# zju3dv/NeuralRecon-W

Hardware: AMD Instinct MI355X
Metric: ray-samples/sec (train step) at 1024 rays x 128 samples (higher is better)
Workload: dtype f16; 1 GPU; brandenburg_gate config (BASELINE.json configs[1]): 1024 rays/GPU x (64 coarse + 64 fine) samples, SDF 8x256 + colour 4x256 + bg NeRF 8x256, 4 outside samples, up_sample_steps 2, render+loss+backward+allreduce+clip+Adam; rays_per_gpu=1024, samples_per_ray=128, global_rays=1024, parallelism=dp1, world_size=1, submission=eager, streams=2, skipped_steps=0

## Files before the change

### neuralrecon-w_amd/csrc/ncw_split.hip

```cpp
#include "ncw_mlp.h"

#ifdef NCW_HALF_F16

namespace {

constexpr int SS_WAVES = 8, SS_TILES = 4;
constexpr int SS_ACT = SS_TILES * 16 * 2 * 1024;
constexpr int SS_GAM = SS_TILES * 3 * 2 * 1024;
constexpr int SB_ACT = SS_TILES * 16 * 1024;

typedef __attribute__((address_space(3))) bf16x8 ss_lfrag;

NCW_DEV bf16x8 ss_gload(const void* w, size_t unit, int lane) {
    return ncw_ld_frag<bf16x8>(w, (size_t)unit, lane);
}

template <int NU>
NCW_DEV void ss_load_half(bf16x8 (&h)[NU], bf16x8 (&l)[NU], const void* w, const void* wlo, int rb_stride, int ob, int u0, int lane) {
#pragma unroll
    for (int q = 0; q < NU; ++q) {
        h[q] = ss_gload(w, (size_t)(u0 + q) * rb_stride + ob, lane);
        l[q] = ss_gload(wlo, (size_t)(u0 + q) * rb_stride + ob, lane);
    }
}

NCW_DEV void ss_split8(const f32x16& v, int t, bf16x8& hi, bf16x8& lo) { ncw_split8(v, t, hi, lo); }

constexpr int SS_RD = 2;
template <int NU>
NCW_DEV void ss_mma(f32x16 (&acc)[SS_TILES], const bf16x8 (&wh)[NU], const bf16x8 (&wl)[NU], const ss_lfrag* in, int upt, int u0) {
    constexpr int NS = (SS_TILES / 2) * NU, RD = SS_RD < NS ? SS_RD : NS, R = RD + 1 < NS ? RD + 1 : NS;
    bf16x8 b[R][4];
    auto ring_read = [&](int s) {
        const ss_lfrag* p0 = in + ((2 * (s / NU) * upt + u0 + s % NU) * 2) * 64;
        const ss_lfrag* p1 = in + (((2 * (s / NU) + 1) * upt + u0 + s % NU) * 2) * 64;
        b[s % R][0] = p0[0]; b[s % R][1] = p0[64];
        b[s % R][2] = p1[0]; b[s % R][3] = p1[64];
    };
#pragma unroll
    for (int s = 0; s < RD; ++s) ring_read(s);
#pragma unroll
    for (int s = 0; s < NS; ++s) {
        if (s + RD < NS) ring_read(s + RD);
        const int tp = 2 * (s / NU), q = s % NU;
        const bf16x8 (&f)[4] = b[s % R];
        acc[tp] = NCW_MFMA_H(wh[q], f[0], acc[tp], 0, 0, 0);
        acc[tp + 1] = NCW_MFMA_H(wh[q], f[2], acc[tp + 1], 0, 0, 0);
        acc[tp] = NCW_MFMA_H(wl[q], f[0], acc[tp], 0, 0, 0);
        acc[tp + 1] = NCW_MFMA_H(wl[q], f[2], acc[tp + 1], 0, 0, 0);
        acc[tp] = NCW_MFMA_H(wh[q], f[1], acc[tp], 0, 0, 0);
        acc[tp + 1] = NCW_MFMA_H(wh[q], f[3], acc[tp + 1], 0, 0, 0);
        __builtin_amdgcn_sched_barrier(0);
    }
}

NCW_DEV f32x16 ss_bias(const float* bp, int ob, int lane) {
    CVec<1> b1;
    load_bias(b1, bp + ob * 32, lane);
    return b1.v[0];
}

NCW_DEV void ss_load_sprime(f32x16& sv, const ncw_h16* __restrict__ st_h, size_t tile, int RB, int rb, int lane) {
    stash_load_block(sv, st_h, tile, RB, rb, lane);
#pragma unroll
    for (int r = 0; r < 16; ++r) sv[r] = 1.f - __builtin_amdgcn_exp2f(sv[r] * -144.26950408889634f);
}

template <int STASH>
NCW_DEV void ss_value_chain(const NcwSdfNet& net, const NcwPoints& src, int64_t n, int64_t tile0, ss_lfrag* abuf, ss_lfrag* gbuf,
                            int lane, int wave, float* __restrict__ sdf, const NcwSdfStash& st) {
    typedef ncw_h16 SE;
    constexpr bool TU = STASH == 0;
    const float bscale = TU ? NCW_TU : 1.f;
    const int L = net.n_layers;
    if (wave < SS_TILES) {
        int64_t p = (tile0 + wave) * 32 + (lane & 31), ray;
        if (p >= n) p = n - 1;
        float xs[3];
        load_point(src, p, xs, ray);
        xs[0] *= net.scale; xs[1] *= net.scale; xs[2] *= net.scale;
        CVec<2> gam;
        freq_encode<2, 3, 6, false>(gam, xs, lane);
        if (STASH == 2) stash_store<2>((SE*)st.gamma, (size_t)(tile0 + wave), gam, lane);
        if (TU) cvec_scale<2>(gam, NCW_TU);
#pragma unroll
        for (int q = 0; q < 3; ++q) {
            bf16x8 hi, lo;
            ss_split8(gam.v[q >> 1], q & 1, hi, lo);
            gbuf[((wave * 3 + q) * 2 + 0) * 64 + lane] = hi;
            gbuf[((wave * 3 + q) * 2 + 1) * 64 + lane] = lo;
        }
    }
    bf16x8 Ah[8], Al[8], Bh[8], Bl[8];
    f32x16 acc[SS_TILES];
    const ss_lfrag* const ain = abuf + lane;
    const ss_lfrag* const gin = gbuf + lane;
    auto epilogue = [&](int l_out) {
        ncw_lds_barrier();
#pragma unroll
        for (int t = 0; t < SS_TILES; ++t) {
            f32x16 yv;
#pragma unroll
            for (int r = 0; r < 16; ++r) yv[r] = softplus_sel<TU>(acc[t][r]);
            if (STASH >= 1) stash_store_block_keep((SE*)st.h[l_out], (size_t)(tile0 + t), 8, wave, yv, lane);
#pragma unroll
            for (int tt = 0; tt < 2; ++tt) {
                bf16x8 hi, lo;
                ss_split8(yv, tt, hi, lo);
                abuf[((t * 16 + 2 * wave + tt) * 2 + 0) * 64 + lane] = hi;
                abuf[((t * 16 + 2 * wave + tt) * 2 + 1) * 64 + lane] = lo;
            }
        }
        ncw_lds_barrier();
    };
    f32x16 bnext;
    {
        bf16x8 w0h[3], w0l[3];
        ss_load_half<3>(w0h, w0l, net.w[0], net.w_lo[0], 8, wave, 0, lane);
        if (L - 1 > 1) ss_load_half<8>(Ah, Al, net.w[1], net.w_lo[1], 8, wave, 0, lane);
        const f32x16 bias = ss_bias(net.b[0], wave, lane) * bscale;
#pragma unroll
        for (int t = 0; t < SS_TILES; ++t) acc[t] = bias;
        ncw_lds_barrier();
        ss_mma<3>(acc, w0h, w0l, gin, 3, 0);
        bnext = ss_bias(net.b[L - 1 > 1 ? 1 : 0], wave, lane);
        epilogue(1);
    }
    for (int l = 1; l < L - 1; ++l) {
        const f32x16 bias = bnext * bscale;
#pragma unroll
        for (int t = 0; t < SS_TILES; ++t) acc[t] = bias;
        ss_load_half<8>(Bh, Bl, net.w[l], net.w_lo[l], 8, wave, 8, lane);
        ss_mma<8>(acc, Ah, Al, ain, 16, 0);
        if (l + 1 < L - 1) ss_load_half<8>(Ah, Al, net.w[l + 1], net.w_lo[l + 1], 8, wave, 0, lane);
        ss_mma<8>(acc, Bh, Bl, ain, 16, 8);
        if (l == net.skip_layer) {
            bf16x8 wgh[3], wgl[3];
            ss_load_half<3>(wgh, wgl, net.w[l], net.w_lo[l], 8, wave, 16, lane);
            ss_mma<3>(acc, wgh, wgl, gin, 3, 0);
        }
        bnext = ss_bias(net.b[l + 1 < L - 1 ? l + 1 : l], wave, lane);
        epilogue(l + 1);
    }
    if (wave < SS_TILES) {
        CVec<1> o;
        load_bias(o, net.b[L - 1], lane);
        if (TU) cvec_scale<1>(o, NCW_TU);
#pragma unroll
        for (int half = 0; half < 2; ++half) {
            bf16x8 wh[8], wl[8];
            ss_load_half<8>(wh, wl, net.w[L - 1], net.w_lo[L - 1], 1, 0, 8 * half, lane);
#pragma unroll
            for (int q = 0; q < 8; ++q) {
                const ss_lfrag* p = ain + ((wave * 16 + 8 * half + q) * 2) * 64;
                const bf16x8 bh = p[0], bl = p[64];
                o.v[0] = NCW_MFMA_H(wh[q], bh, o.v[0], 0, 0, 0);
                o.v[0] = NCW_MFMA_H(wl[q], bh, o.v[0], 0, 0, 0);
                o.v[0] = NCW_MFMA_H(wh[q], bl, o.v[0], 0, 0, 0);
            }
        }
        const int64_t p = (tile0 + wave) * 32 + (lane & 31);
        if (p < n && lane < 32) sdf[p] = o.v[0][0] / (net.scale * bscale);
    }
}

constexpr int S2_TILE = 16 * 2 * 1024;

constexpr int S2_BIAS = 8 * 1024;
typedef __attribute__((address_space(3))) f32x4 ss_lf4;

NCW_DEV void s2_barrier() {
    asm volatile("s_waitcnt lgkmcnt(0)" ::: "memory");
    __builtin_amdgcn_s_barrier();
    asm volatile("" ::: "memory");
}

NCW_DEV f32x16 s2_bias(const ss_lf4* bb, int lane) {
    const ss_lf4* p = bb + (lane >> 5) * 4;
    f32x16 v;
#pragma unroll
    for (int g = 0; g < 4; ++g) {
        const f32x4 t = p[g];
#pragma unroll
        for (int c = 0; c < 4; ++c) v[4 * g + c] = t[c];
    }
    return v;
}

template <int NU>
NCW_DEV void s2_mma_x(f32x16& a, const bf16x8* wh, const bf16x8* wl, const ss_lfrag* xin) {
#pragma unroll
    for (int u = 0; u < NU; ++u) {
        const bf16x8 bh = xin[(u * 2) * 64], bl = xin[(u * 2 + 1) * 64];
        a = NCW_MFMA_H(wh[u], bh, a, 0, 0, 0);
        a = NCW_MFMA_H(wl[u], bh, a, 0, 0, 0);
        a = NCW_MFMA_H(wh[u], bl, a, 0, 0, 0);
    }
}

constexpr int S2_RING = 3;
template <bool PREFETCH, class EPI>
NCW_DEV void s2_segment(f32x16& m, bf16x8 (&wh)[16], bf16x8 (&wl)[16], const ss_lfrag* in, const void* wn, const void* wn_lo, int ob,
                        int lane, EPI&& epi) {
    f32x16 c;
#pragma unroll
    for (int r = 0; r < 16; ++r) c[r] = 0.f;
    constexpr int RD = S2_RING - 1;
    bf16x8 b[S2_RING][2];
#pragma unroll
    for (int q = 0; q < RD; ++q) { b[q][0] = in[(q * 2) * 64]; b[q][1] = in[(q * 2 + 1) * 64]; }
#pragma unroll
    for (int u = 0; u < 16; ++u) {
        if (u + RD < 16) {
            b[(u + RD) % S2_RING][0] = in[((u + RD) * 2) * 64];
            b[(u + RD) % S2_RING][1] = in[((u + RD) * 2 + 1) * 64];
        }
        m = NCW_MFMA_H(wh[u], b[u % S2_RING][0], m, 0, 0, 0);
        c = NCW_MFMA_H(wl[u], b[u % S2_RING][0], c, 0, 0, 0);
        c = NCW_MFMA_H(wh[u], b[u % S2_RING][1], c, 0, 0, 0);
        if (PREFETCH) {
            wh[u] = ss_gload(wn, (size_t)u * 8 + ob, lane);
            wl[u] = ss_gload(wn_lo, (size_t)u * 8 + ob, lane);
        }
        epi(u);
        __builtin_amdgcn_sched_barrier(0);
    }
#pragma unroll
    for (int r = 0; r < 16; ++r) m[r] += c[r];
}

template <bool STASH>
NCW_DEV void s2_epi_step(int u, const f32x16& e, bf16x8& fh, bf16x8& fl, float& ycarry, ss_lfrag* out, int ob, int lane,
                         ncw_h16* __restrict__ st_h, size_t tile) {
    const float y = softplus_sel<!STASH>(e[u]);
    if ((u & 1) == 0) {
        ycarry = y;
    } else {
        ncw_h16 h0, h1, l0, l1;
        ncw_split2(ycarry, y, h0, h1, l0, l1);
        fh[(u & 7) - 1] = h0; fh[u & 7] = h1;
        fl[(u & 7) - 1] = l0; fl[u & 7] = l1;
    }
    if (STASH && (u & 3) == 3) {
        bf16x4 t;
#pragma unroll
        for (int c = 0; c < 4; ++c) t[c] = fh[(u & 7) - 3 + c];
        reinterpret_cast<bf16x4*>(st_h)[((tile * 8 + ob) * 4 + (u >> 2)) * 64 + lane] = t;
    }
    if ((u & 7) == 7) {
        const int unit = 2 * ob + (u >> 3);
        out[(unit * 2 + 0) * 64 + lane] = fh;
        out[(unit * 2 + 1) * 64 + lane] = fl;
    }
}

template <bool STASH>
NCW_DEV void s2_value_chain(const NcwSdfNet& net, const NcwPoints& src, int64_t n, int64_t tile0, ss_lfrag* abuf, ss_lfrag* gbuf,
                            ss_lf4* bbuf, int lane, int wave, float* __restrict__ sdf, const NcwSdfStash& st) {
    typedef ncw_h16 SE;
    const int L = net.n_layers, NL = L - 1;
    const int ob = wave;
    constexpr bool TU = !STASH;
    const float bscale = TU ? NCW_TU : 1.f;
    for (int i = threadIdx.x; i < NL * 64; i += 64 * SS_WAVES) bbuf[i] = reinterpret_cast<const f32x4*>(net.b[i >> 6])[i & 63] * bscale;
    if (wave < SS_TILES) {
        int64_t p = (tile0 + wave) * 32 + (lane & 31), ray;
        if (p >= n) p = n - 1;
        float xs[3];
        load_point(src, p, xs, ray);
        xs[0] *= net.scale; xs[1] *= net.scale; xs[2] *= net.scale;
        CVec<2> gam;
        freq_encode<2, 3, 6, false>(gam, xs, lane);
        if (STASH == 2) stash_store<2>((SE*)st.gamma, (size_t)(tile0 + wave), gam, lane);
        if (TU) cvec_scale<2>(gam, NCW_TU);
#pragma unroll
        for (int q = 0; q < 3; ++q) {
            bf16x8 hi, lo;
            ss_split8(gam.v[q >> 1], q & 1, hi, lo);
            gbuf[((wave * 3 + q) * 2 + 0) * 64 + lane] = hi;
            gbuf[((wave * 3 + q) * 2 + 1) * 64 + lane] = lo;
        }
    }
    bf16x8 wh[16], wl[16];
    f32x16 x, y;
    bf16x8 fh, fl;
    float yc = 0.f;
    auto region = [&](int t) { return abuf + t * (S2_TILE / 16); };
    auto gin = [&](int t) { return gbuf + t * 3 * 2 * 64 + lane; };
    auto bias_of = [&](int l) { return s2_bias(bbuf + (l * 8 + ob) * 8, lane); };
    {
        ss_load_half<3>(reinterpret_cast<bf16x8(&)[3]>(wh[0]), reinterpret_cast<bf16x8(&)[3]>(wl[0]), net.w[0], net.w_lo[0], 8, ob, 0, lane);
        s2_barrier();
        x = bias_of(0);
        y = x;
        s2_mma_x<3>(x, wh, wl, gin(0));
        s2_mma_x<3>(y, wh, wl, gin(1));
#pragma unroll
        for (int u = 0; u < 16; ++u) s2_epi_step<STASH>(u, x, fh, fl, yc, region(0), ob, lane, (SE*)st.h[1], (size_t)tile0);
#pragma unroll
        for (int u = 0; u < 16; ++u) s2_epi_step<STASH>(u, y, fh, fl, yc, region(1), ob, lane, (SE*)st.h[1], (size_t)(tile0 + 1));
        x = bias_of(0);
        y = x;
        s2_mma_x<3>(x, wh, wl, gin(2));
        s2_mma_x<3>(y, wh, wl, gin(3));
        if (NL > 1) ss_load_half<16>(wh, wl, net.w[1], net.w_lo[1], 8, ob, 0, lane);
#pragma unroll
        for (int u = 0; u < 16; ++u) s2_epi_step<STASH>(u, x, fh, fl, yc, region(2), ob, lane, (SE*)st.h[1], (size_t)(tile0 + 2));
        s2_barrier();
    }
    for (int l = 1; l < NL; ++l) {
        const bool more = l + 1 < NL, skip = (l == net.skip_layer);
        bf16x8 gh[3], gl[3];
        if (skip) ss_load_half<3>(gh, gl, net.w[l], net.w_lo[l], 8, ob, 16, lane);
        {
            x = bias_of(l);
            auto epi = [&](int u) { s2_epi_step<STASH>(u, y, fh, fl, yc, region(3), ob, lane, (SE*)st.h[l], (size_t)(tile0 + 3)); };
            s2_segment<false>(x, wh, wl, region(0) + lane, nullptr, nullptr, ob, lane, epi);
            if (skip) s2_mma_x<3>(x, gh, gl, gin(0));
            s2_barrier();
        }
        {
            y = bias_of(l);
            auto epi = [&](int u) { s2_epi_step<STASH>(u, x, fh, fl, yc, region(0), ob, lane, (SE*)st.h[l + 1], (size_t)tile0); };
            s2_segment<false>(y, wh, wl, region(1) + lane, nullptr, nullptr, ob, lane, epi);
            if (skip) s2_mma_x<3>(y, gh, gl, gin(1));
            s2_barrier();
        }
        {
            x = bias_of(l);
            auto epi = [&](int u) { s2_epi_step<STASH>(u, y, fh, fl, yc, region(1), ob, lane, (SE*)st.h[l + 1], (size_t)(tile0 + 1)); };
            s2_segment<false>(x, wh, wl, region(2) + lane, nullptr, nullptr, ob, lane, epi);
            if (skip) s2_mma_x<3>(x, gh, gl, gin(2));
            s2_barrier();
        }
        {
            y = bias_of(l);
            auto epi = [&](int u) { s2_epi_step<STASH>(u, x, fh, fl, yc, region(2), ob, lane, (SE*)st.h[l + 1], (size_t)(tile0 + 2)); };
            s2_segment<true>(y, wh, wl, region(3) + lane, more ? net.w[l + 1] : net.w[l], more ? net.w_lo[l + 1] : net.w_lo[l], ob, lane, epi);
            if (skip) s2_mma_x<3>(y, gh, gl, gin(3));
            s2_barrier();
        }
    }
#pragma unroll
    for (int u = 0; u < 16; ++u) s2_epi_step<STASH>(u, y, fh, fl, yc, region(3), ob, lane, (SE*)st.h[NL], (size_t)(tile0 + 3));
    s2_barrier();
    if (wave < SS_TILES) {
        CVec<1> o;
        load_bias(o, net.b[L - 1], lane);
        if (TU) cvec_scale<1>(o, NCW_TU);
        const ss_lfrag* in = region(wave) + lane;
#pragma unroll
        for (int half = 0; half < 2; ++half) {
            bf16x8 vh[8], vl[8];
            ss_load_half<8>(vh, vl, net.w[L - 1], net.w_lo[L - 1], 1, 0, 8 * half, lane);
#pragma unroll
            for (int q = 0; q < 8; ++q) {
                const ss_lfrag* p = in + ((8 * half + q) * 2) * 64;
                const bf16x8 bh = p[0], bl = p[64];
                o.v[0] = NCW_MFMA_H(vh[q], bh, o.v[0], 0, 0, 0);
                o.v[0] = NCW_MFMA_H(vl[q], bh, o.v[0], 0, 0, 0);
                o.v[0] = NCW_MFMA_H(vh[q], bl, o.v[0], 0, 0, 0);
            }
        }
        const int64_t p = (tile0 + wave) * 32 + (lane & 31);
        if (p < n && lane < 32) sdf[p] = o.v[0][0] / (net.scale * bscale);
    }
}

__global__ __launch_bounds__(64 * SS_WAVES) void sdf_inferS2_kernel(NcwSdfNet net, NcwPoints src, int64_t n,
                                                                   float* __restrict__ sdf) {
    __shared__ __attribute__((aligned(16))) char lds[SS_ACT + SS_GAM + S2_BIAS];
    ss_lfrag* const abuf = (ss_lfrag*)(ncw_lchar*)lds;
    ss_lfrag* const gbuf = abuf + SS_ACT / 16;
    ss_lf4* const bbuf = (ss_lf4*)(gbuf + SS_GAM / 16);
    const int lane = ncw_lane();
    const int wave = __builtin_amdgcn_readfirstlane((int)(threadIdx.x >> 6));
    NcwSdfStash none = {};
    s2_value_chain<false>(net, src, n, (int64_t)blockIdx.x * SS_TILES, abuf, gbuf, bbuf, lane, wave, sdf, none);
}

__global__ __launch_bounds__(64 * SS_WAVES) void sdf_inferS_kernel(NcwSdfNet net, NcwPoints src, int64_t n,
                                                                  float* __restrict__ sdf) {
    __shared__ __attribute__((aligned(16))) char lds[SS_ACT + SS_GAM];
    ss_lfrag* const abuf = (ss_lfrag*)(ncw_lchar*)lds;
    ss_lfrag* const gbuf = abuf + SS_ACT / 16;
    const int lane = ncw_lane();
    const int wave = __builtin_amdgcn_readfirstlane((int)(threadIdx.x >> 6));
    NcwSdfStash none = {};
    ss_value_chain<0>(net, src, n, (int64_t)blockIdx.x * SS_TILES, abuf, gbuf, lane, wave, sdf, none);
}

typedef __attribute__((address_space(3))) bf16x8 sb_lfrag;

template <int NU>
NCW_DEV void sb_load_slice(bf16x8* a, const void* w, int rb_stride, int ob, int u0, int lane) {
#pragma unroll
    for (int q = 0; q < NU; ++q) a[q] = ss_gload(w, (size_t)(u0 + q) * rb_stride + ob, lane);
}

NCW_DEV void sb_store_units(sb_lfrag* buf, int t, int ob, const f32x16& v, int lane) {
    Act<PrecBF16, 1> o;
    to_act_block<1>(o, 0, v);
    buf[(t * 16 + 2 * ob) * 64 + lane] = o.f[0];
    buf[(t * 16 + 2 * ob + 1) * 64 + lane] = o.f[1];
}

NCW_DEV float ss_gamma_deriv(float x0, float x1, float x2, int f, int& comp) {
    if (f < 3) {
        comp = f;
        return 1.f;
    }
    if (f >= 3 * (2 * 6 + 1)) {
        comp = 0;
        return 0.f;
    }
    const int j = f - 3;
    const int k = j / 6;
    const int rem = j - k * 6;
    const bool is_cos = rem >= 3;
    comp = is_cos ? rem - 3 : rem;
    const float v = comp == 2 ? x2 : (comp == 1 ? x1 : x0);
    const float fr = (float)(1 << k);
    const float arg = v * fr;
    return is_cos ? -fr * sinf(arg) : fr * cosf(arg);
}

NCW_DEV float ss_sprime(ncw_h16 h) { return 1.f - __builtin_amdgcn_exp2f((float)h * -144.26950408889634f); }

NCW_DEV void ss_request_h(bf16x4 (&raw)[4], const ncw_h16* __restrict__ st_h, size_t tile, int RB, int rb, int lane) {
    const bf16x4* p = reinterpret_cast<const bf16x4*>(st_h) + ((tile * RB + rb) * 4) * 64 + lane;
#pragma unroll
    for (int g = 0; g < 4; ++g) raw[g] = NCW_STASH_LD(p[g * 64]);
}

template <bool TRAIN>
NCW_DEV void ss_sweep_start(ss_lfrag* sbuf, const f32x16& a0, ncw_h16* __restrict__ st_t, size_t tile0, int wave, int lane) {
    bf16x8 hf[SS_TILES][2];
#pragma unroll
    for (int t = 0; t < SS_TILES; ++t)
#pragma unroll
        for (int tt = 0; tt < 2; ++tt) hf[t][tt] = sbuf[((t * 16 + 2 * wave + tt) * 2) * 64 + lane];
    ncw_lds_barrier();
    sb_lfrag* out = (sb_lfrag*)sbuf;
#pragma unroll
    for (int t = 0; t < SS_TILES; ++t) {
        f32x16 sv;
#pragma unroll
        for (int r = 0; r < 16; ++r) sv[r] = ss_sprime(hf[t][r >> 3][r & 7]) * a0[r];
        if (TRAIN) stash_store_block(st_t, tile0 + t, 8, wave, sv, lane);
        sb_store_units(out, t, wave, sv, lane);
    }
}

constexpr int SA_RD = 2;
template <int NW, int STEP, bool RELOAD>
NCW_DEV void sa_mma(f32x16& acc0, f32x16& acc1, bf16x8 (&w0)[16], bf16x8 (&w1)[16], const sb_lfrag* in0, const sb_lfrag* in1,
                    const void* n0 = nullptr, const void* n1 = nullptr, int nstride = 0, int ob = 0, int lane = 0) {
    constexpr int RD = SA_RD, R = RD + 1;
    bf16x8 b[R][2];
    const char* p0 = (const char*)n0 + (size_t)ob * 1024;
    const char* p1 = (const char*)n1 + (size_t)ob * 1024;
    const size_t pstep = (size_t)nstride * 1024;
    auto reload = [&](int u) {
        asm volatile("" : "+s"(p0), "+s"(p1));
        w0[u] = ss_gload(p0, 0, lane);
        if (NW == 2) w1[u] = ss_gload(p1, 0, lane);
        p0 += pstep;
        p1 += pstep;
    };
#pragma unroll
    for (int q = 0; q < RD; ++q) { b[q][0] = in0[q * STEP]; b[q][1] = in1[q * STEP]; }
#pragma unroll
    for (int u = 0; u < 16; ++u) {
        if (RELOAD && u >= 1) reload(u - 1);
        if (u + RD < 16) { b[(u + RD) % R][0] = in0[(u + RD) * STEP]; b[(u + RD) % R][1] = in1[(u + RD) * STEP]; }
        acc0 = NCW_MFMA_H(w0[u], b[u % R][0], acc0, 0, 0, 0);
        acc1 = NCW_MFMA_H(w0[u], b[u % R][1], acc1, 0, 0, 0);
        if (NW == 2) {
            acc0 = NCW_MFMA_H(w1[u], b[u % R][0], acc0, 0, 0, 0);
            acc1 = NCW_MFMA_H(w1[u], b[u % R][1], acc1, 0, 0, 0);
        }
        __builtin_amdgcn_sched_barrier(0);
    }
    if (RELOAD) reload(15);
}

template <bool TRAIN>
__global__ __launch_bounds__(64 * SS_WAVES) void sdf_fwdS_kernel(NcwSdfNet net, NcwPoints src, int64_t n,
                                                                float* __restrict__ sdf, float* __restrict__ grad,
                                                                NcwSdfStash st) {
    typedef ncw_h16 SE;
    __shared__ __attribute__((aligned(16))) char lds[SS_ACT + SS_GAM];
    ss_lfrag* const sbuf = (ss_lfrag*)(ncw_lchar*)lds;
    ss_lfrag* const gbuf = sbuf + SS_ACT / 16;
    const int lane = ncw_lane();
    const int wave = __builtin_amdgcn_readfirstlane((int)(threadIdx.x >> 6));
    const int L = net.n_layers;
    const int64_t tile0 = (int64_t)blockIdx.x * SS_TILES;
    const int jb = wave & 1, jt = wave >> 1;
    ss_value_chain<(TRAIN ? 2 : 1)>(net, src, n, tile0, sbuf, gbuf, lane, wave, sdf, st);
    bf16x8 wa[16], wb[16];
    {
        sb_load_slice<16>(wa, net.w_feat, 8, wave, 0, lane);
        const bf16x8 wt1 = ss_gload(net.wt[L - 1], (size_t)wave, lane);
        if (L - 2 >= 1) sb_load_slice<16>(wb, net.wt[L - 2], (L - 2 == net.skip_layer) ? 10 : 8, wave, 0, lane);
        const f32x16 bias = ss_bias(net.b_feat, wave, lane);
        const ss_lfrag* const ain = sbuf + lane;
#pragma unroll
        for (int tp = 0; tp < SS_TILES; tp += 2) {
            f32x16 acc0 = bias, acc1 = bias;
#pragma unroll
            for (int q = 0; q < 16; ++q) {
                acc0 = NCW_MFMA_H(wa[q], ain[((tp * 16 + q) * 2) * 64], acc0, 0, 0, 0);
                acc1 = NCW_MFMA_H(wa[q], ain[(((tp + 1) * 16 + q) * 2) * 64], acc1, 0, 0, 0);
            }
            stash_store_block((SE*)st.feat, (size_t)(tile0 + tp), 8, wave, acc0, lane);
            stash_store_block((SE*)st.feat, (size_t)(tile0 + tp + 1), 8, wave, acc1, lane);
        }
        bf16x8 e0f;
#pragma unroll
        for (int e = 0; e < 8; ++e) e0f[e] = (ncw_h16)0.f;
        e0f[0] = (ncw_h16)(lane < 32 ? 1.f : 0.f);
        f32x16 a0;
#pragma unroll
        for (int r = 0; r < 16; ++r) a0[r] = 0.f;
        a0 = NCW_MFMA_H(wt1, e0f, a0, 0, 0, 0);
        ss_sweep_start<TRAIN>(sbuf, a0, (SE*)st.t[L - 2], (size_t)tile0, wave, lane);
#pragma unroll
        for (int q = 0; q < 16; ++q) wa[q] = wb[q];
    }
    sb_lfrag* const abuf0 = (sb_lfrag*)sbuf;
    sb_lfrag* const abuf1 = abuf0 + SB_ACT / 16;
    int cur = 0;
    f32x16 gg;
#pragma unroll
    for (int r = 0; r < 16; ++r) gg[r] = 0.f;
    for (int l = L - 2; l >= 1; --l) {
        const bool skip = (l == net.skip_layer);
        if (!skip && l - 1 >= 1) sb_load_slice<16>(wb, net.wt[l - 1], (l - 1 == net.skip_layer) ? 10 : 8, wave, 0, lane);
        ncw_lds_barrier();
        const sb_lfrag* in = cur ? abuf1 : abuf0;
        sb_lfrag* out = cur ? abuf0 : abuf1;
#pragma unroll
        for (int tp = 0; tp < SS_TILES; tp += 2) {
            f32x16 acc0, acc1;
#pragma unroll
            for (int r = 0; r < 16; ++r) { acc0[r] = 0.f; acc1[r] = 0.f; }
#pragma unroll
            for (int q = 0; q < 16; ++q) {
                acc0 = NCW_MFMA_H(wa[q], in[(tp * 16 + q) * 64 + lane], acc0, 0, 0, 0);
                acc1 = NCW_MFMA_H(wa[q], in[((tp + 1) * 16 + q) * 64 + lane], acc1, 0, 0, 0);
            }
#pragma unroll
            for (int j = 0; j < 2; ++j) {
                const f32x16& acc = j ? acc1 : acc0;
                f32x16 sv;
                ss_load_sprime(sv, (const SE*)st.h[l], (size_t)(tile0 + tp + j), 8, wave, lane);
#pragma unroll
                for (int r = 0; r < 16; ++r) sv[r] *= acc[r];
                if (TRAIN) stash_store_block((SE*)st.t[l - 1], (size_t)(tile0 + tp + j), 8, wave, sv, lane);
                sb_store_units(out, tp + j, wave, sv, lane);
            }
        }
        if (skip) {
            sb_load_slice<16>(wb, net.wt[l], 10, 8 + jb, 0, lane);
#pragma unroll
            for (int q = 0; q < 16; ++q) gg = NCW_MFMA_H(wb[q], in[(jt * 16 + q) * 64 + lane], gg, 0, 0, 0);
            if (l - 1 >= 1) sb_load_slice<16>(wb, net.wt[l - 1], (l - 1 == net.skip_layer) ? 10 : 8, wave, 0, lane);
        }
#pragma unroll
        for (int q = 0; q < 16; ++q) wa[q] = wb[q];
        cur ^= 1;
    }
    sb_load_slice<16>(wb, net.wt[0], 2, jb, 0, lane);
    ncw_lds_barrier();
    {
        const sb_lfrag* in = cur ? abuf1 : abuf0;
#pragma unroll
        for (int q = 0; q < 16; ++q) gg = NCW_MFMA_H(wb[q], in[(jt * 16 + q) * 64 + lane], gg, 0, 0, 0);
    }
    int64_t p = (tile0 + jt) * 32 + (lane & 31), ray;
    const bool valid = p < n;
    if (!valid) p = n - 1;
    float xs[3];
    load_point(src, p, xs, ray);
    xs[0] *= net.scale; xs[1] *= net.scale; xs[2] *= net.scale;
    float nx = 0.f, ny = 0.f, nz = 0.f;
    const int h = lane >> 5;
#pragma unroll
    for (int r = 0; r < 16; ++r) {
        const int f0 = 32 * jb + ncw_feat_of(r, 0);
        if (f0 >= 39) continue;
        int comp;
        const float dv = freq_feature_deriv<3, 6, true>(xs, f0 + 4 * h, comp);
        const float c = gg[r] * dv;
        nx += comp == 0 ? c : 0.f;
        ny += comp == 1 ? c : 0.f;
        nz += comp == 2 ? c : 0.f;
    }
    nx = half_pair_sum(nx); ny = half_pair_sum(ny); nz = half_pair_sum(nz);
    typedef __attribute__((address_space(3))) float lfloat;
    lfloat* part = (lfloat*)gbuf;
    if (jb == 1 && lane < 32) {
        part[(jt * 32 + lane) * 3 + 0] = nx; part[(jt * 32 + lane) * 3 + 1] = ny; part[(jt * 32 + lane) * 3 + 2] = nz;
    }
    ncw_lds_barrier();
    if (jb == 0 && lane < 32 && valid) {
        grad[p * 3 + 0] = nx + part[(jt * 32 + lane) * 3 + 0];
        grad[p * 3 + 1] = ny + part[(jt * 32 + lane) * 3 + 1];
        grad[p * 3 + 2] = nz + part[(jt * 32 + lane) * 3 + 2];
    }
}

template <bool TRAIN>
__global__ __launch_bounds__(64 * SS_WAVES) void sdf_fwdSA_kernel(NcwSdfNet net, NcwPoints src, int64_t n,
                                                                 float* __restrict__ sdf, float* __restrict__ grad,
                                                                 NcwSdfStash st) {
    typedef ncw_h16 SE;
    __shared__ __attribute__((aligned(16))) char lds[SS_ACT + SS_GAM];
    ss_lfrag* const sbuf = (ss_lfrag*)(ncw_lchar*)lds;
    ss_lfrag* const gbuf = sbuf + SS_ACT / 16;
    const int lane = ncw_lane();
    const int wave = __builtin_amdgcn_readfirstlane((int)(threadIdx.x >> 6));
    const int L = net.n_layers;
    const int64_t tile0 = (int64_t)blockIdx.x * SS_TILES;
    const int jb = wave & 1, jt = wave >> 1;
    ss_value_chain<(TRAIN ? 2 : 1)>(net, src, n, tile0, sbuf, gbuf, lane, wave, sdf, st);
    auto stride_of = [&](int l) { return l == net.skip_layer ? 10 : (l == 0 ? 2 : 8); };
    bf16x8 wa[16], wl[16];
    {
        sb_load_slice<16>(wl, net.w_feat, 8, wave, 0, lane);
        const bf16x8 wt1 = ss_gload(net.wt[L - 1], (size_t)wave, lane);
        const bf16x8 wt1l = ss_gload(net.wt_lo[L - 1], (size_t)wave, lane);
        if (L - 2 >= 1) sb_load_slice<16>(wa, net.wt[L - 2], stride_of(L - 2), wave, 0, lane);
        const f32x16 bias = ss_bias(net.b_feat, wave, lane);
        const sb_lfrag* const ain = (const sb_lfrag*)sbuf + lane;
#pragma unroll
        for (int tp = 0; tp < SS_TILES; tp += 2) {
            f32x16 acc0 = bias, acc1 = bias;
            const sb_lfrag* in0 = ain + (tp * 16 * 2) * 64;
            const sb_lfrag* in1 = ain + ((tp + 1) * 16 * 2) * 64;
            if (tp == SS_TILES - 2) sa_mma<1, 2 * 64, true>(acc0, acc1, wl, wl, in0, in1, net.wt_lo[L - 2], nullptr, stride_of(L - 2), wave, lane);
            else sa_mma<1, 2 * 64, false>(acc0, acc1, wl, wl, in0, in1);
            stash_store_block((SE*)st.feat, (size_t)(tile0 + tp), 8, wave, acc0, lane);
            stash_store_block((SE*)st.feat, (size_t)(tile0 + tp + 1), 8, wave, acc1, lane);
        }
        bf16x8 e0f;
#pragma unroll
        for (int e = 0; e < 8; ++e) e0f[e] = (ncw_h16)0.f;
        e0f[0] = (ncw_h16)(lane < 32 ? 1.f : 0.f);
        f32x16 a0;
#pragma unroll
        for (int r = 0; r < 16; ++r) a0[r] = 0.f;
        a0 = NCW_MFMA_H(wt1, e0f, a0, 0, 0, 0);
        a0 = NCW_MFMA_H(wt1l, e0f, a0, 0, 0, 0);
        ss_sweep_start<TRAIN>(sbuf, a0, (SE*)st.t[L - 2], (size_t)tile0, wave, lane);
    }
    sb_lfrag* const abuf0 = (sb_lfrag*)sbuf;
    sb_lfrag* const abuf1 = abuf0 + SB_ACT / 16;
    int cur = 0;
    f32x16 gg;
#pragma unroll
    for (int r = 0; r < 16; ++r) gg[r] = 0.f;
    auto gamma_job = [&](const void* w, const void* wlo, int stride, int ob, const sb_lfrag* in) {
#pragma unroll
        for (int c = 0; c < 2; ++c) {
            bf16x8 th[8], tl[8];
            sb_load_slice<8>(th, w, stride, ob, 8 * c, lane);
            sb_load_slice<8>(tl, wlo, stride, ob, 8 * c, lane);
            __builtin_amdgcn_sched_barrier(0);
#pragma unroll
            for (int q = 0; q < 8; ++q) {
                const bf16x8 b = in[(jt * 16 + 8 * c + q) * 64 + lane];
                gg = NCW_MFMA_H(th[q], b, gg, 0, 0, 0);
                gg = NCW_MFMA_H(tl[q], b, gg, 0, 0, 0);
            }
        }
    };
    for (int l = L - 2; l >= 1; --l) {
        const bool skip = (l == net.skip_layer);
        const int ln = l - 1 >= 1 ? l - 1 : l;
        const void* nh = net.wt[ln];
        const void* nl = net.wt_lo[ln];
        const int nstride = stride_of(ln);
        ncw_lds_barrier();
        const sb_lfrag* in = cur ? abuf1 : abuf0;
        sb_lfrag* out = cur ? abuf0 : abuf1;
#pragma unroll
        for (int tp = 0; tp < SS_TILES; tp += 2) {
            f32x16 acc0, acc1;
#pragma unroll
            for (int r = 0; r < 16; ++r) { acc0[r] = 0.f; acc1[r] = 0.f; }
            const sb_lfrag* in0 = in + (tp * 16) * 64 + lane;
            const sb_lfrag* in1 = in + ((tp + 1) * 16) * 64 + lane;
            bf16x4 hr[2][4];
            ss_request_h(hr[0], (const SE*)st.h[l], (size_t)(tile0 + tp), 8, wave, lane);
            ss_request_h(hr[1], (const SE*)st.h[l], (size_t)(tile0 + tp + 1), 8, wave, lane);
            if (tp == SS_TILES - 2) sa_mma<2, 64, true>(acc0, acc1, wa, wl, in0, in1, nh, nl, nstride, wave, lane);
            else sa_mma<2, 64, false>(acc0, acc1, wa, wl, in0, in1);
#pragma unroll
            for (int j = 0; j < 2; ++j) {
                const f32x16& acc = j ? acc1 : acc0;
                f32x16 sv;
#pragma unroll
                for (int r = 0; r < 16; ++r) sv[r] = ss_sprime(hr[j][r >> 2][r & 3]) * acc[r];
                if (TRAIN) stash_store_block((SE*)st.t[l - 1], (size_t)(tile0 + tp + j), 8, wave, sv, lane);
                sb_store_units(out, tp + j, wave, sv, lane);
            }
        }
        if (skip) gamma_job(net.wt[l], net.wt_lo[l], 10, 8 + jb, in);
        cur ^= 1;
    }
    ncw_lds_barrier();
    gamma_job(net.wt[0], net.wt_lo[0], 2, jb, cur ? abuf1 : abuf0);
    int64_t p = (tile0 + jt) * 32 + (lane & 31), ray;
    const bool valid = p < n;
    if (!valid) p = n - 1;
    float xs[3];
    load_point(src, p, xs, ray);
    xs[0] *= net.scale; xs[1] *= net.scale; xs[2] *= net.scale;
    float nx = 0.f, ny = 0.f, nz = 0.f;
    const int h = lane >> 5;
#pragma unroll
    for (int r = 0; r < 16; ++r) {
        const int f0 = 32 * jb + ncw_feat_of(r, 0);
        if (f0 >= 39) continue;
        int comp;
        const float dv = ss_gamma_deriv(xs[0], xs[1], xs[2], f0 + 4 * h, comp);
        const float c = gg[r] * dv;
        nx += comp == 0 ? c : 0.f;
        ny += comp == 1 ? c : 0.f;
        nz += comp == 2 ? c : 0.f;
    }
    nx = half_pair_sum(nx); ny = half_pair_sum(ny); nz = half_pair_sum(nz);
    typedef __attribute__((address_space(3))) float lfloat;
    lfloat* part = (lfloat*)gbuf;
    if (jb == 1 && lane < 32) {
        part[(jt * 32 + lane) * 3 + 0] = nx; part[(jt * 32 + lane) * 3 + 1] = ny; part[(jt * 32 + lane) * 3 + 2] = nz;
    }
    ncw_lds_barrier();
    if (jb == 0 && lane < 32 && valid) {
        grad[p * 3 + 0] = nx + part[(jt * 32 + lane) * 3 + 0];
        grad[p * 3 + 1] = ny + part[(jt * 32 + lane) * 3 + 1];
        grad[p * 3 + 2] = nz + part[(jt * 32 + lane) * 3 + 2];
    }
}

constexpr int NS_WAVES = 8, NS_TILES = 2;
constexpr int NS_ACT = NS_TILES * 16 * 2 * 1024;
constexpr int NS_X = NS_TILES * 6 * 2 * 1024;

NCW_DEV void ns_inverted_sphere(const float (&x)[3], float (&p4)[4]) {
    float r = sqrtf(x[0] * x[0] + x[1] * x[1] + x[2] * x[2]);
    r = fminf(fmaxf(r, 1.0f), 1e10f);
    p4[0] = x[0] / r; p4[1] = x[1] / r; p4[2] = x[2] / r; p4[3] = 1.0f / r;
}

template <int NU>
NCW_DEV void ns_mma(f32x16 (&acc)[NS_TILES], const bf16x8 (&wh)[NU], const bf16x8 (&wl)[NU], const ss_lfrag* in, int upt, int iu0) {
#pragma unroll
    for (int q = 0; q < NU; ++q) {
        const ss_lfrag* p0 = in + ((0 * upt + iu0 + q) * 2) * 64;
        const ss_lfrag* p1 = in + ((1 * upt + iu0 + q) * 2) * 64;
        const bf16x8 bh0 = p0[0], bl0 = p0[64], bh1 = p1[0], bl1 = p1[64];
        acc[0] = NCW_MFMA_H(wh[q], bh0, acc[0], 0, 0, 0);
        acc[1] = NCW_MFMA_H(wh[q], bh1, acc[1], 0, 0, 0);
        acc[0] = NCW_MFMA_H(wl[q], bh0, acc[0], 0, 0, 0);
        acc[1] = NCW_MFMA_H(wl[q], bh1, acc[1], 0, 0, 0);
        acc[0] = NCW_MFMA_H(wh[q], bl0, acc[0], 0, 0, 0);
        acc[1] = NCW_MFMA_H(wh[q], bl1, acc[1], 0, 0, 0);
    }
}
template <int NU>
NCW_DEV void ns_mma1(f32x16& acc, const bf16x8 (&wh)[NU], const bf16x8 (&wl)[NU], const ss_lfrag* in, int t, int upt, int iu0) {
#pragma unroll
    for (int q = 0; q < NU; ++q) {
        const ss_lfrag* p0 = in + ((t * upt + iu0 + q) * 2) * 64;
        const bf16x8 bh = p0[0], bl = p0[64];
        acc = NCW_MFMA_H(wh[q], bh, acc, 0, 0, 0);
        acc = NCW_MFMA_H(wl[q], bh, acc, 0, 0, 0);
        acc = NCW_MFMA_H(wh[q], bl, acc, 0, 0, 0);
    }
}

NCW_DEV void ns_store(ss_lfrag* abuf, int t, int ob, const f32x16& v, int lane) {
#pragma unroll
    for (int tt = 0; tt < 2; ++tt) {
        bf16x8 hi, lo;
        ss_split8(v, tt, hi, lo);
        abuf[((t * 16 + 2 * ob + tt) * 2 + 0) * 64 + lane] = hi;
        abuf[((t * 16 + 2 * ob + tt) * 2 + 1) * 64 + lane] = lo;
    }
}

__global__ __launch_bounds__(64 * NS_WAVES) void nerf_refineS_kernel(NcwNerfNet net, NcwPoints src, int64_t n, const float* __restrict__ aux_bias,
                                                                    float* __restrict__ density, float* __restrict__ rgb) {
    __shared__ __attribute__((aligned(16))) char lds[NS_ACT + NS_X + NS_TILES * 32 * 4];
    ss_lfrag* const abuf = (ss_lfrag*)(ncw_lchar*)lds;
    ss_lfrag* const xbuf = abuf + NS_ACT / 16;
    typedef __attribute__((address_space(3))) int ns_lint;
    ns_lint* const rbuf = (ns_lint*)(xbuf + NS_X / 16);
    const int lane = ncw_lane();
    const int wave = __builtin_amdgcn_readfirstlane((int)(threadIdx.x >> 6));
    const int64_t tile0 = (int64_t)blockIdx.x * NS_TILES;
    const int D = net.D;
    n = points_count(src, n);
    if (tile0 * 32 >= n) return;
    int64_t pp = 0;
    bool pvalid = false;
    if (wave < NS_TILES) {
        int64_t p = (tile0 + wave) * 32 + (lane & 31), ray;
        pvalid = p < n;
        if (!pvalid) p = n - 1;
        pp = point_slot(src, p);
        float xs[3], p4[4];
        load_point(src, p, xs, ray);
        ns_inverted_sphere(xs, p4);
        if (lane < 32) rbuf[wave * 32 + lane] = (int)ray;
        CVec<3> gp;
        freq_encode<3, 4, 10, false>(gp, p4, lane);
#pragma unroll
        for (int q = 0; q < 6; ++q) {
            bf16x8 hi, lo;
            ss_split8(gp.v[q >> 1], q & 1, hi, lo);
            xbuf[((wave * 6 + q) * 2 + 0) * 64 + lane] = hi;
            xbuf[((wave * 6 + q) * 2 + 1) * 64 + lane] = lo;
        }
    }
    bf16x8 Ah[8], Al[8], Bh[8], Bl[8];
    f32x16 acc[NS_TILES];
    const ss_lfrag* const ain = abuf + lane;
    const ss_lfrag* const xin = xbuf + lane;
    auto relu_store = [&](int ob) {
        ncw_lds_barrier();
#pragma unroll
        for (int t = 0; t < NS_TILES; ++t) {
            f32x16 y;
#pragma unroll
            for (int r = 0; r < 16; ++r) y[r] = ncw_relu(acc[t][r]);
            ns_store(abuf, t, ob, y, lane);
        }
        ncw_lds_barrier();
    };
    {
        bf16x8 w0h[6], w0l[6];
        ss_load_half<6>(w0h, w0l, net.w_p[0], net.w_p_lo[0], 8, wave, 0, lane);
        if (D > 1) ss_load_half<8>(Ah, Al, net.w_p[1], net.w_p_lo[1], 8, wave, 0, lane);
        const f32x16 bias = ss_bias(net.b_p[0], wave, lane);
        acc[0] = bias; acc[1] = bias;
        ncw_lds_barrier();
        ns_mma<6>(acc, w0h, w0l, xin, 6, 0);
        relu_store(wave);
    }
    for (int i = 1; i < D; ++i) {
        const f32x16 bias = ss_bias(net.b_p[i], wave, lane);
        acc[0] = bias; acc[1] = bias;
        ss_load_half<8>(Bh, Bl, net.w_p[i], net.w_p_lo[i], 8, wave, 8, lane);
        ns_mma<8>(acc, Ah, Al, ain, 16, 0);
        {
            const void* nh = i + 1 < D ? net.w_p[i + 1] : net.w_feat;
            const void* nl = i + 1 < D ? net.w_p_lo[i + 1] : net.w_feat_lo;
            ss_load_half<8>(Ah, Al, nh, nl, 8, wave, 0, lane);
        }
        ns_mma<8>(acc, Bh, Bl, ain, 16, 8);
        if (i == net.skip + 1) {
            bf16x8 wgh[6], wgl[6];
            ss_load_half<6>(wgh, wgl, net.w_p[i], net.w_p_lo[i], 8, wave, 16, lane);
            ns_mma<6>(acc, wgh, wgl, xin, 6, 0);
        }
        relu_store(wave);
    }
    if (wave < NS_TILES) {
        CVec<1> o;
        load_bias(o, net.b_alpha, lane);
#pragma unroll
        for (int half = 0; half < 2; ++half) {
            bf16x8 wh[8], wl[8];
            ss_load_half<8>(wh, wl, net.w_alpha, net.w_alpha_lo, 1, 0, 8 * half, lane);
            ns_mma1<8>(o.v[0], wh, wl, ain, wave, 16, 8 * half);
        }
        if (pvalid && lane < 32) density[pp] = o.v[0][0];
    }
    {
        const f32x16 bias = ss_bias(net.b_feat, wave, lane);
        acc[0] = bias; acc[1] = bias;
        ss_load_half<8>(Bh, Bl, net.w_feat, net.w_feat_lo, 8, wave, 8, lane);
        ns_mma<8>(acc, Ah, Al, ain, 16, 0);
        ns_mma<8>(acc, Bh, Bl, ain, 16, 8);
        ncw_lds_barrier();
#pragma unroll
        for (int t = 0; t < NS_TILES; ++t) ns_store(abuf, t, wave, acc[t], lane);
        ncw_lds_barrier();
    }
    const int hb = wave & 3, ht = wave >> 2;
    f32x16 hacc;
    {
        hacc = ss_bias(net.b_a[0], hb, lane);
        ncw_add_ray_bias_block(hacc, aux_bias + (size_t)rbuf[ht * 32 + (lane & 31)] * 128, hb, lane);
#pragma unroll
        for (int half = 0; half < 2; ++half) {
            bf16x8 wh[8], wl[8];
            ss_load_half<8>(wh, wl, net.w_a[0], net.w_a_lo[0], 4, hb, 8 * half, lane);
            ns_mma1<8>(hacc, wh, wl, ain, ht, 16, 8 * half);
        }
        ncw_lds_barrier();
        f32x16 y;
#pragma unroll
        for (int r = 0; r < 16; ++r) y[r] = ncw_relu(hacc[r]);
        ns_store(abuf, ht, hb, y, lane);
        ncw_lds_barrier();
    }
    for (int i = 1; i < net.n_head; ++i) {
        hacc = ss_bias(net.b_a[i], hb, lane);
        bf16x8 wh[8], wl[8];
        ss_load_half<8>(wh, wl, net.w_a[i], net.w_a_lo[i], 4, hb, 0, lane);
        ns_mma1<8>(hacc, wh, wl, ain, ht, 16, 0);
        ncw_lds_barrier();
        f32x16 y;
#pragma unroll
        for (int r = 0; r < 16; ++r) y[r] = ncw_relu(hacc[r]);
        ns_store(abuf, ht, hb, y, lane);
        ncw_lds_barrier();
    }
    if (wave < NS_TILES) {
        CVec<1> o;
        load_bias(o, net.b_rgb, lane);
        bf16x8 wh[8], wl[8];
        ss_load_half<8>(wh, wl, net.w_rgb, net.w_rgb_lo, 1, 0, 0, lane);
        ns_mma1<8>(o.v[0], wh, wl, ain, wave, 16, 0);
        if (pvalid && lane < 32) {
            rgb[pp * 3 + 0] = o.v[0][0];
            rgb[pp * 3 + 1] = o.v[0][1];
            rgb[pp * 3 + 2] = o.v[0][2];
        }
    }
}

}

int ncw_sdf_inferS_launch_f16(const NcwSdfNet* net, const NcwPoints& src, int64_t n, float* sdf, hipStream_t st) {
    const int64_t tiles = (n + 31) / 32;
    const dim3 grid((unsigned)((tiles + SS_TILES - 1) / SS_TILES));
    if (net->n_layers - 1 <= 8) {
        hipLaunchKernelGGL(sdf_inferS2_kernel, grid, dim3(64 * SS_WAVES), 0, st, *net, src, n, sdf);
    } else hipLaunchKernelGGL(sdf_inferS_kernel, grid, dim3(64 * SS_WAVES), 0, st, *net, src, n, sdf);
    NCW_CHECK_LAUNCH();
    return 0;
}

int ncw_sdf_fwdS_launch_f16(const NcwSdfNet* net, const NcwPoints& src, int64_t n, float* sdf, float* grad,
                            const NcwSdfStash& stash, hipStream_t st) {
    const int64_t tiles = (n + 31) / 32;
    const dim3 grid((unsigned)((tiles + SS_TILES - 1) / SS_TILES));
    bool adj = net->n_layers >= 3;
    for (int l = 0; l < net->n_layers; ++l) adj = adj && net->wt_lo[l] != nullptr;
    const bool render = stash.t[0] == nullptr;
    if (adj) {
        if (render) hipLaunchKernelGGL(sdf_fwdSA_kernel<false>, grid, dim3(64 * SS_WAVES), 0, st, *net, src, n, sdf, grad, stash);
        else hipLaunchKernelGGL(sdf_fwdSA_kernel<true>, grid, dim3(64 * SS_WAVES), 0, st, *net, src, n, sdf, grad, stash);
    } else {
        if (render) hipLaunchKernelGGL(sdf_fwdS_kernel<false>, grid, dim3(64 * SS_WAVES), 0, st, *net, src, n, sdf, grad, stash);
        else hipLaunchKernelGGL(sdf_fwdS_kernel<true>, grid, dim3(64 * SS_WAVES), 0, st, *net, src, n, sdf, grad, stash);
    }
    NCW_CHECK_LAUNCH();
    return 0;
}

int ncw_nerf_refineS_launch_f16(const NcwNerfNet* net, const NcwPoints& src, int64_t n, const float* aux_bias, float* density,
                                float* rgb, hipStream_t st) {
    const int64_t tiles = (n + 31) / 32;
    hipLaunchKernelGGL(nerf_refineS_kernel, dim3((unsigned)((tiles + NS_TILES - 1) / NS_TILES)), dim3(64 * NS_WAVES), 0, st, *net, src,
                       n, aux_bias, density, rgb);
    NCW_CHECK_LAUNCH();
    return 0;
}

#endif
```

Measured before the change: 32.67 million ray-samples/s.

## Pipeline SDF forward value chain with in-place ping-pong tiles and overlapped epilogue

Adds a new value-chain routine for the training forward kernels. It processes tile pairs in a ping-pong across two LDS regions, so the softplus/split epilogue and the stash stores for one pair run interleaved with the MFMAs of the other pair. Next-layer weights are reloaded incrementally inside the MMA loop, and biases are prefetched and published through a small LDS buffer. The aim is to hide epilogue, global-load and barrier latency behind matrix work, at the cost of extra LDS, higher register pressure and more complex scheduling.

```diff
diff --git a/neuralrecon-w_amd/csrc/ncw_split.hip b/neuralrecon-w_amd/csrc/ncw_split.hip
--- a/neuralrecon-w_amd/csrc/ncw_split.hip
+++ b/neuralrecon-w_amd/csrc/ncw_split.hip
@@ -22,6 +22,12 @@
         h[q] = ss_gload(w, (size_t)(u0 + q) * rb_stride + ob, lane);
         l[q] = ss_gload(wlo, (size_t)(u0 + q) * rb_stride + ob, lane);
     }
+}
+
+template <int NU>
+NCW_DEV void sb_load_slice(bf16x8* a, const void* w, int rb_stride, int ob, int u0, int lane) {
+#pragma unroll
+    for (int q = 0; q < NU; ++q) a[q] = ss_gload(w, (size_t)(u0 + q) * rb_stride + ob, lane);
 }
 
 NCW_DEV void ss_split8(const f32x16& v, int t, bf16x8& hi, bf16x8& lo) { ncw_split8(v, t, hi, lo); }
@@ -367,6 +373,197 @@
     }
 }
 
+constexpr int SP_BIAS = SS_WAVES * 32 * 4;
+typedef __attribute__((address_space(3))) float ss_lf1;
+
+NCW_DEV unsigned sp_lane_off(int lane, unsigned bytes) {
+    unsigned off = (unsigned)lane * bytes;
+    asm volatile("" : "+v"(off));
+    return off;
+}
+NCW_DEV bf16x8 sp_gload(const char* p, int lane) {
+    typedef const __attribute__((address_space(1))) bf16x8* gp;
+    return *(gp)(p + sp_lane_off(lane, 16));
+}
+NCW_DEV void sp_epi_step(int u, const f32x16& e0, const f32x16& e1, bf16x8& fh, bf16x8& fl, ss_lfrag* out0, int ob, int lane,
+                         ncw_h16* __restrict__ st_h, size_t tile) {
+    const int j = u >> 3, k = u & 7, el = (2 * k) & 7;
+    const f32x16& e = j ? e1 : e0;
+    ncw_h16 h0, h1, l0, l1;
+    ncw_split2(softplus_sel<false>(e[2 * k]), softplus_sel<false>(e[2 * k + 1]), h0, h1, l0, l1);
+    fh[el] = h0; fh[el + 1] = h1;
+    fl[el] = l0; fl[el + 1] = l1;
+    if (k & 1) {
+        bf16x4 t;
+#pragma unroll
+        for (int c = 0; c < 4; ++c) t[c] = fh[el - 2 + c];
+        typedef __attribute__((address_space(1))) bf16x4* gp;
+        char* base = (char*)st_h + (((tile + j) * 8 + ob) * 4 + (k >> 1)) * (64 * sizeof(bf16x4));
+        *(gp)(base + sp_lane_off(lane, sizeof(bf16x4))) = t;
+    }
+    if ((k & 3) == 3) {
+        ss_lfrag* out = out0 + j * (SS_ACT / SS_TILES / 16);
+        const int unit = 2 * ob + (k >> 2);
+        out[(unit * 2 + 0) * 64 + lane] = fh;
+        out[(unit * 2 + 1) * 64 + lane] = fl;
+    }
+}
+
+template <bool RELOAD, class EPI>
+NCW_DEV void sp_stage(f32x16& a0, f32x16& a1, bf16x8 (&wh)[16], bf16x8 (&wl)[16], const ss_lfrag* in0, const ss_lfrag* in1,
+                      const void* n0, const void* n1, int ob, int lane, EPI&& epi) {
+    bf16x8 b[2][4];
+    const char* p0 = (const char*)n0 + (size_t)ob * 1024;
+    const char* p1 = (const char*)n1 + (size_t)ob * 1024;
+    auto reload = [&](int u) {
+        asm volatile("" : "+s"(p0), "+s"(p1));
+        wh[u] = sp_gload(p0, lane);
+        wl[u] = sp_gload(p1, lane);
+        p0 += 8 * 1024;
+        p1 += 8 * 1024;
+    };
+    auto ring_read = [&](int s) {
+        b[s & 1][0] = in0[(s * 2) * 64]; b[s & 1][1] = in0[(s * 2 + 1) * 64];
+        b[s & 1][2] = in1[(s * 2) * 64]; b[s & 1][3] = in1[(s * 2 + 1) * 64];
+    };
+    ring_read(0);
+#pragma unroll
+    for (int u = 0; u < 16; ++u) {
+        if (RELOAD && u >= 1) reload(u - 1);
+        if (u + 1 < 16) ring_read(u + 1);
+        const bf16x8 (&f)[4] = b[u & 1];
+        a0 = NCW_MFMA_H(wh[u], f[0], a0, 0, 0, 0);
+        a1 = NCW_MFMA_H(wh[u], f[2], a1, 0, 0, 0);
+        a0 = NCW_MFMA_H(wl[u], f[0], a0, 0, 0, 0);
+        a1 = NCW_MFMA_H(wl[u], f[2], a1, 0, 0, 0);
+        a0 = NCW_MFMA_H(wh[u], f[1], a0, 0, 0, 0);
+        a1 = NCW_MFMA_H(wh[u], f[3], a1, 0, 0, 0);
+        epi(u);
+        __builtin_amdgcn_sched_barrier(0);
+    }
+}
+
+template <class TAIL>
+NCW_DEV void sp_gamma(f32x16& a0, f32x16& a1, const void* w, const void* wlo, int ob, int lane, const ss_lfrag* xin, TAIL&& tail) {
+    bf16x8 gh[3], gl[3];
+    ss_load_half<3>(gh, gl, w, wlo, 8, ob, 16, lane);
+    __builtin_amdgcn_sched_barrier(0);
+    tail();
+    __builtin_amdgcn_sched_barrier(0);
+#pragma unroll
+    for (int q = 0; q < 3; ++q) {
+        const bf16x8 f0 = xin[(q * 2) * 64], f1 = xin[(q * 2 + 1) * 64];
+        const bf16x8 f2 = xin[((3 + q) * 2) * 64], f3 = xin[((3 + q) * 2 + 1) * 64];
+        a0 = NCW_MFMA_H(gh[q], f0, a0, 0, 0, 0);
+        a1 = NCW_MFMA_H(gh[q], f2, a1, 0, 0, 0);
+        a0 = NCW_MFMA_H(gl[q], f0, a0, 0, 0, 0);
+        a1 = NCW_MFMA_H(gl[q], f2, a1, 0, 0, 0);
+        a0 = NCW_MFMA_H(gh[q], f1, a0, 0, 0, 0);
+        a1 = NCW_MFMA_H(gh[q], f3, a1, 0, 0, 0);
+    }
+}
+
+template <int STASH>
+NCW_DEV void sp_value_chain(const NcwSdfNet& net, const NcwPoints& src, int64_t n, int64_t tile0, ss_lfrag* abuf, ss_lfrag* gbuf,
+                            ss_lf1* bbuf, int lane, int wave, float* __restrict__ sdf, const NcwSdfStash& st) {
+    typedef ncw_h16 SE;
+    const int L = net.n_layers, NL = L - 1;
+    const int ob = wave;
+    if (wave < SS_TILES) {
+        int64_t p = (tile0 + wave) * 32 + (lane & 31), ray;
+        if (p >= n) p = n - 1;
+        float xs[3];
+        load_point(src, p, xs, ray);
+        xs[0] *= net.scale; xs[1] *= net.scale; xs[2] *= net.scale;
+        CVec<2> gam;
+        freq_encode<2, 3, 6, false>(gam, xs, lane);
+        if (STASH == 2) stash_store<2>((SE*)st.gamma, (size_t)(tile0 + wave), gam, lane);
+#pragma unroll
+        for (int q = 0; q < 3; ++q) {
+            bf16x8 hi, lo;
+            ss_split8(gam.v[q >> 1], q & 1, hi, lo);
+            gbuf[((wave * 3 + q) * 2 + 0) * 64 + lane] = hi;
+            gbuf[((wave * 3 + q) * 2 + 1) * 64 + lane] = lo;
+        }
+    }
+    bf16x8 wh[16], wl[16];
+    f32x16 acc[SS_TILES];
+    bf16x8 fh, fl;
+    auto region = [&](int t) { return abuf + t * (SS_ACT / SS_TILES / 16); };
+    ss_lf1* const bmine = bbuf + ob * 32;
+    auto bias_request = [&](int l) { return net.b[l][ob * 32 + (lane & 31)]; };
+    auto bias_publish = [&](float v) { bmine[lane & 31] = v; };
+    auto bias_read = [&]() { return s2_bias((const ss_lf4*)bmine, lane); };
+    {
+        bf16x8 w0h[3], w0l[3];
+        ss_load_half<3>(w0h, w0l, net.w[0], net.w_lo[0], 8, ob, 0, lane);
+        const f32x16 bias = ss_bias(net.b[0], ob, lane);
+        const float b1 = bias_request(NL > 1 ? 1 : 0);
+#pragma unroll
+        for (int t = 0; t < SS_TILES; ++t) acc[t] = bias;
+        s2_barrier();
+        ss_mma<3>(acc, w0h, w0l, gbuf + lane, 3, 0);
+        bias_publish(b1);
+        if (NL > 1) ss_load_half<16>(wh, wl, net.w[1], net.w_lo[1], 8, ob, 0, lane);
+#pragma unroll
+        for (int u = 0; u < 16; ++u) sp_epi_step(u, acc[0], acc[1], fh, fl, region(0), ob, lane, (SE*)st.h[1], (size_t)tile0);
+        s2_barrier();
+    }
+    for (int l = 1; l < NL; ++l) {
+        const bool skip = (l == net.skip_layer);
+        const int ln = l + 1 < NL ? l + 1 : l;
+        float bn;
+        {
+            acc[0] = bias_read();
+            acc[1] = acc[0];
+            auto epi = [&](int u) { sp_epi_step(u, acc[2], acc[3], fh, fl, region(2), ob, lane, (SE*)st.h[l], (size_t)(tile0 + 2)); };
+            sp_stage<false>(acc[0], acc[1], wh, wl, region(0) + lane, region(1) + lane, nullptr, nullptr, ob, lane, epi);
+            auto tail = [&]() { bn = bias_request(ln); };
+            if (skip) sp_gamma(acc[0], acc[1], net.w[l], net.w_lo[l], ob, lane, gbuf + lane, tail);
+            else tail();
+            s2_barrier();
+        }
+        {
+            acc[2] = bias_read();
+            acc[3] = acc[2];
+            auto epi = [&](int u) { sp_epi_step(u, acc[0], acc[1], fh, fl, region(0), ob, lane, (SE*)st.h[l + 1], (size_t)tile0); };
+            sp_stage<true>(acc[2], acc[3], wh, wl, region(2) + lane, region(3) + lane, net.w[ln], net.w_lo[ln], ob, lane, epi);
+            auto tail = [&]() {
+                wh[15] = ss_gload(net.w[ln], (size_t)15 * 8 + ob, lane);
+                wl[15] = ss_gload(net.w_lo[ln], (size_t)15 * 8 + ob, lane);
+            };
+            if (skip) sp_gamma(acc[2], acc[3], net.w[l], net.w_lo[l], ob, lane, gbuf + 2 * 3 * 2 * 64 + lane, tail);
+            else tail();
+            bias_publish(bn);
+            s2_barrier();
+        }
+    }
+#pragma unroll
+    for (int u = 0; u < 16; ++u) sp_epi_step(u, acc[2], acc[3], fh, fl, region(2), ob, lane, (SE*)st.h[NL], (size_t)(tile0 + 2));
+    asm volatile("s_waitcnt vmcnt(0)" ::: "memory");
+    s2_barrier();
+    if (wave < SS_TILES) {
+        CVec<1> o;
+        load_bias(o, net.b[L - 1], lane);
+        const ss_lfrag* in = region(wave) + lane;
+#pragma unroll
+        for (int half = 0; half < 2; ++half) {
+            bf16x8 vh[8], vl[8];
+            ss_load_half<8>(vh, vl, net.w[L - 1], net.w_lo[L - 1], 1, 0, 8 * half, lane);
+#pragma unroll
+            for (int q = 0; q < 8; ++q) {
+                const ss_lfrag* p = in + ((8 * half + q) * 2) * 64;
+                const bf16x8 bh = p[0], bl = p[64];
+                o.v[0] = NCW_MFMA_H(vh[q], bh, o.v[0], 0, 0, 0);
+                o.v[0] = NCW_MFMA_H(vl[q], bh, o.v[0], 0, 0, 0);
+                o.v[0] = NCW_MFMA_H(vh[q], bl, o.v[0], 0, 0, 0);
+            }
+        }
+        const int64_t p = (tile0 + wave) * 32 + (lane & 31);
+        if (p < n && lane < 32) sdf[p] = o.v[0][0] / net.scale;
+    }
+}
+
 __global__ __launch_bounds__(64 * SS_WAVES) void sdf_inferS2_kernel(NcwSdfNet net, NcwPoints src, int64_t n,
                                                                    float* __restrict__ sdf) {
     __shared__ __attribute__((aligned(16))) char lds[SS_ACT + SS_GAM + S2_BIAS];
@@ -391,12 +588,6 @@
 }
 
 typedef __attribute__((address_space(3))) bf16x8 sb_lfrag;
-
-template <int NU>
-NCW_DEV void sb_load_slice(bf16x8* a, const void* w, int rb_stride, int ob, int u0, int lane) {
-#pragma unroll
-    for (int q = 0; q < NU; ++q) a[q] = ss_gload(w, (size_t)(u0 + q) * rb_stride + ob, lane);
-}
 
 NCW_DEV void sb_store_units(sb_lfrag* buf, int t, int ob, const f32x16& v, int lane) {
     Act<PrecBF16, 1> o;
@@ -490,15 +681,16 @@
                                                                 float* __restrict__ sdf, float* __restrict__ grad,
                                                                 NcwSdfStash st) {
     typedef ncw_h16 SE;
-    __shared__ __attribute__((aligned(16))) char lds[SS_ACT + SS_GAM];
+    __shared__ __attribute__((aligned(16))) char lds[SS_ACT + SS_GAM + SP_BIAS];
     ss_lfrag* const sbuf = (ss_lfrag*)(ncw_lchar*)lds;
     ss_lfrag* const gbuf = sbuf + SS_ACT / 16;
+    ss_lf1* const bbuf = (ss_lf1*)(gbuf + SS_GAM / 16);
     const int lane = ncw_lane();
     const int wave = __builtin_amdgcn_readfirstlane((int)(threadIdx.x >> 6));
     const int L = net.n_layers;
     const int64_t tile0 = (int64_t)blockIdx.x * SS_TILES;
     const int jb = wave & 1, jt = wave >> 1;
-    ss_value_chain<(TRAIN ? 2 : 1)>(net, src, n, tile0, sbuf, gbuf, lane, wave, sdf, st);
+    sp_value_chain<(TRAIN ? 2 : 1)>(net, src, n, tile0, sbuf, gbuf, bbuf, lane, wave, sdf, st);
     bf16x8 wa[16], wb[16];
     {
         sb_load_slice<16>(wa, net.w_feat, 8, wave, 0, lane);
@@ -617,15 +809,16 @@
                                                                  float* __restrict__ sdf, float* __restrict__ grad,
                                                                  NcwSdfStash st) {
     typedef ncw_h16 SE;
-    __shared__ __attribute__((aligned(16))) char lds[SS_ACT + SS_GAM];
+    __shared__ __attribute__((aligned(16))) char lds[SS_ACT + SS_GAM + SP_BIAS];
     ss_lfrag* const sbuf = (ss_lfrag*)(ncw_lchar*)lds;
     ss_lfrag* const gbuf = sbuf + SS_ACT / 16;
+    ss_lf1* const bbuf = (ss_lf1*)(gbuf + SS_GAM / 16);
     const int lane = ncw_lane();
     const int wave = __builtin_amdgcn_readfirstlane((int)(threadIdx.x >> 6));
     const int L = net.n_layers;
     const int64_t tile0 = (int64_t)blockIdx.x * SS_TILES;
     const int jb = wave & 1, jt = wave >> 1;
-    ss_value_chain<(TRAIN ? 2 : 1)>(net, src, n, tile0, sbuf, gbuf, lane, wave, sdf, st);
+    sp_value_chain<(TRAIN ? 2 : 1)>(net, src, n, tile0, sbuf, gbuf, bbuf, lane, wave, sdf, st);
     auto stride_of = [&](int l) { return l == net.skip_layer ? 10 : (l == 0 ? 2 : 8); };
     bf16x8 wa[16], wl[16];
     {
```

Measured after the change: 32.89 million ray-samples/s, median of 6. Within noise of the previous version (+0.7%).
